# GmxMahdi/compute-raytracer

Hardware: AMD Instinct MI355X
Metric: Mrays/s at 3840x2160, 1024 spheres, 8 bounces (higher is better)
Workload: dtype f32; 1 GPU; C3: 3840x2160, 1024 spheres (seed 358), 8 bounces, constant sky, reference default camera/light; mode=fast, variant=0, rays_per_frame=46143642, frames_in_flight=4, parallelism=row-tiles x1

## Files before the change

### compute_raytracer_amd/csrc/rt_bvh.hip

```cpp
#include <algorithm>
#include <cmath>
#include <cstdlib>
#include <vector>

#include "rt_filter.h"

#define RT_BVH_KAPPA 6.103515625e-05f
#define RT_BVH_REV_DELTA 0.0051f
#define RT_BVH_REV_DELTA_REL 7.62939453125e-06f
#define RT_BVH_REV_SLACK 2.44140625e-04f
#define RT_BVH_REV_SLACK_ABS 4.76837158203125e-07f

#ifndef RT_BVH_GRAB
#define RT_BVH_GRAB 256u
#endif
#ifndef RT_BVH_TAIL_SMALL
#define RT_BVH_TAIL_SMALL 16
#endif
#ifndef RT_BVH_TAIL_SERIAL
#define RT_BVH_TAIL_SERIAL 12
#endif
#ifndef RT_BVH_TAIL_LARGE
#define RT_BVH_TAIL_LARGE 28
#endif

namespace rtk {

__host__ __device__ inline uint32_t bvh_lds_l0(uint32_t n_nodes, uint32_t base) {
    uint32_t l0 = 1024u;
    const uint32_t need = (4u * (n_nodes + 1u) + 2u) / 3u;
    if (base + l0 < need) l0 = need - base;
    return (l0 + 15u) & ~15u;
}
__host__ __device__ inline uint32_t bvh_gap_waves(uint32_t n_nodes, uint32_t waves) {
    const uint32_t k = (bvh_lds_l0(n_nodes, 0u) - 1024u) / 512u;
    return k < waves ? k : waves;
}
__host__ __device__ constexpr uint32_t bvh_list_bytes(bool nlds, uint32_t cap) { return nlds ? 128u * (cap + 1u) : 256u * cap; }
__host__ __device__ inline uint32_t bvh_lds_lists(uint32_t n_nodes, uint32_t base) {
    const uint32_t l0 = bvh_lds_l0(n_nodes, base);
    return 4u * (base + l0) - base + 16u * ((n_nodes + 4u) & ~3u);
}

__global__ void bvh_fill_leaves(float4* rec, const uint32_t* link, uint32_t n_nodes, const float4* geo_f) {
    const uint32_t i = blockIdx.x * blockDim.x + threadIdx.x;
    if (i >= n_nodes) return;
    const uint32_t l = link[i];
    if (l & 0x80000000u) rec[i] = geo_f[l & 0x7FFFFFFFu];
}

__device__ __forceinline__ double wave_max_f64(double v) {
#pragma unroll
    for (int off = 32; off > 0; off >>= 1) v = fmax(v, __shfl_xor(v, off, 64));
    return v;
}
__device__ __forceinline__ double wave_min_f64(double v) {
#pragma unroll
    for (int off = 32; off > 0; off >>= 1) v = fmin(v, __shfl_xor(v, off, 64));
    return v;
}

__global__ __launch_bounds__(256) void bvh_refit(float4* __restrict__ rec, const uint32_t* __restrict__ link,
                                                  uint32_t n_nodes, const float* __restrict__ records) {
    const uint32_t node = blockIdx.x * 4u + (threadIdx.x >> 6), lane = threadIdx.x & 63u;
    if (node >= n_nodes) return;
    const uint32_t lk = link[node];
    if (lk & 0x80000000u) return;
    const uint32_t first = node + 1u, end = lk >> 2;
    auto sphere = [&](uint32_t j, double c[3], double& r) -> bool {
        if (j >= end) return false;
        const uint32_t l = link[j];
        if (!(l & 0x80000000u)) return false;
        const float* s = records + 8u * (size_t)(l & 0x7FFFFFFFu);
        for (int a = 0; a < 3; ++a) { const double v = (double)s[a]; c[a] = v == v ? v : 0.0; }
        const double rv = fabs((double)s[7]);
        r = rv == rv ? rv : 0.0;
        return true;
    };
    auto radius_at = [&](const double P[3], double far[3]) -> double {
        double best = -1.0, bc[3] = {0.0, 0.0, 0.0};
        for (uint32_t j = first + lane; j < end; j += 64u) {
            double c[3], r;
            if (!sphere(j, c, r)) continue;
            const double dx = c[0] - P[0], dy = c[1] - P[1], dz = c[2] - P[2];
            const double d = sqrt(dx * dx + dy * dy + dz * dz) + r;
            if (d > best) { best = d; bc[0] = c[0]; bc[1] = c[1]; bc[2] = c[2]; }
        }
        const double R = wave_max_f64(best);
        const uint64_t who = __ballot(best == R);
        const int src = who ? (int)__builtin_ctzll(who) : 0;
        for (int a = 0; a < 3; ++a) far[a] = __shfl(bc[a], src, 64);
        return R;
    };
    double mn[3] = {INFINITY, INFINITY, INFINITY}, mx[3] = {-INFINITY, -INFINITY, -INFINITY};
    for (uint32_t j = first + lane; j < end; j += 64u) {
        double c[3], r;
        if (!sphere(j, c, r)) continue;
        for (int a = 0; a < 3; ++a) { mn[a] = fmin(mn[a], c[a] - r); mx[a] = fmax(mx[a], c[a] + r); }
    }
    double P[3];
    for (int a = 0; a < 3; ++a) P[a] = 0.5 * (wave_min_f64(mn[a]) + wave_max_f64(mx[a]));
    double far[3];
    double Rp = radius_at(P, far);
    for (int it = 0; it < 32; ++it) {
        const double sx = far[0] - P[0], sy = far[1] - P[1], sz = far[2] - P[2];
        const double len = sqrt(sx * sx + sy * sy + sz * sz);
        if (!(len > 1e-12)) break;
        const double Q[3] = {P[0] + sx / len * 0.05 * Rp, P[1] + sy / len * 0.05 * Rp, P[2] + sz / len * 0.05 * Rp};
        double farq[3];
        const double Rq = radius_at(Q, farq);
        if (!(Rq < Rp)) break;
        P[0] = Q[0]; P[1] = Q[1]; P[2] = Q[2]; Rp = Rq;
        far[0] = farq[0]; far[1] = farq[1]; far[2] = farq[2];
    }
    const float C[3] = {(float)P[0], (float)P[1], (float)P[2]};
    const double Cd[3] = {(double)C[0], (double)C[1], (double)C[2]};
    double unused[3];
    double R = radius_at(Cd, unused);
    R *= RT_BVH_SIGMA;
    const double c2 = Cd[0] * Cd[0] + Cd[1] * Cd[1] + Cd[2] * Cd[2];
    const double k = c2 * (1.0 - (double)RT_FILTER_EPS) - R * R * (1.0 + (double)RT_FILTER_KAPPA);
    if (lane == 0)
        rec[node] = make_float4(C[0] * RT_FILTER_SCALE, C[1] * RT_FILTER_SCALE, C[2] * RT_FILTER_SCALE,
                                (float)(k * (double)RT_FILTER_SCALE2));
}

#ifdef RT_BVH_COUNT
#define g_steps steps_acc
__device__ unsigned long long g_wave_clock[3 * 8192];
#endif
__device__ __forceinline__ float min0(float b) {
    float d; asm("v_min_f32 %0, 0, %1" : "=v"(d) : "v"(b)); return d;
}

__device__ __forceinline__ void exact_any_order(v3 center, float r2, int s, v3 o, v3 d, float fa, float ta,
                                                float& nearest, int& idx) {
    const v3 oc = sub(o, center);
    const float b = 2.0f * dot(d, oc);
    const float c = dot(oc, oc) - r2;
    const float disc = b * b - fa * c;
    if (disc > 0.0f && b < 0.0f) {
        const float t = (-b - sqrtf(disc)) / ta;
        if (t > 0.001f && (t < nearest || (t == nearest && idx >= 0 && s < idx))) {
            nearest = t;
            idx = s;
        }
    }
}

__device__ __forceinline__ void reversed_shadow_walk(bool shadow, v3 L, float light_l1, v3 P, v3 s, v3& wo, v3& wd, float& madd) {
    const v3 dl = sub(P, L);
    const float l1 = (__builtin_fabsf(dl.x) + __builtin_fabsf(dl.y)) + __builtin_fabsf(dl.z);
    const float la = l1 + light_l1;
    const float delta = __builtin_fmaf(la, RT_BVH_REV_DELTA_REL, RT_BVH_REV_DELTA);
    const float lb = l1 + delta;
    const float slack = __builtin_fmaf(lb * lb, RT_BVH_REV_SLACK, (la * la) * RT_BVH_REV_SLACK_ABS);
    if (shadow) {
        wo = V(__builtin_fmaf(delta, s.x, P.x), __builtin_fmaf(delta, s.y, P.y), __builtin_fmaf(delta, s.z, P.z));
        wd = V(-s.x, -s.y, -s.z);
        madd = slack;
    }
}

#define RT_BVH_DEC_DELTA 0.0050011f
#define RT_BVH_DEC_REL 9.5367431640625e-07f
__device__ __forceinline__ bool shadow_decided(v3 L, float light_l1, v3 s, float len, v3 c, float r2) {
    const float a2 = dot(s, s);
    const v3 oc = sub(L, c);
    const float b = 2.0f * dot(s, oc);
    const float cc = dot(oc, oc) - r2;
    const float disc = b * b - (4.0f * a2) * cc;
    if (!(disc > 0.0f && b < 0.0f)) return false;
    const float tk = (-b - sqrtf(disc)) / (2.0f * a2);
    const float d_a = __builtin_fmaf(len + light_l1, RT_BVH_DEC_REL, RT_BVH_DEC_DELTA);
    const float l_lo = len * (1.0f - RT_BVH_DEC_REL);
    return tk > 0.001f && tk < 9999.0f && tk + d_a <= l_lo;
}

template <bool SGN, bool NLDS, int CAP, bool ROOMY>
__device__ __forceinline__ void trace_bvh(const uint32_t tail, const float4* __restrict__ R, const uint32_t* __restrict__ L, uint32_t n,
                                          const float4* __restrict__ geo, uint32_t* slot, unsigned long long* best,
                                          uint32_t& i, v3 o, v3 d, v3 wo, v3 wd, float madd, float& nearest, int& idx
#ifdef RT_BVH_COUNT
                                          , uint32_t& steps_acc
#endif
                                          ) {
    const float a = dot(wd, wd);
    const float inv = __builtin_amdgcn_rsqf(a) * (1.0f + RT_BVH_KAPPA);
    const v3 h = V(wd.x * inv, wd.y * inv, wd.z * inv);
    const v3 os = V(wo.x * RT_FILTER_SCALE, wo.y * RT_FILTER_SCALE, wo.z * RT_FILTER_SCALE);
    const v3 m = V(-2.0f * os.x, -2.0f * os.y, -2.0f * os.z);
    const float p = dot(h, os);
    const float q = __builtin_fmaf(-madd, RT_FILTER_SCALE2, dot(os, os) * (1.0f - RT_FILTER_EPS));
    constexpr bool CLAMPED = SGN && NLDS;
    constexpr float kT = 2.168404344971009e-19f;
    constexpr float kT2 = 4.70197740328915e-38f;
    const v3 hs = V(h.x * kT, h.y * kT, h.z * kT);
    const v3 ms = V(m.x * kT2, m.y * kT2, m.z * kT2);
    const float ps = -p * kT, qs = q * kT2;
    typedef __attribute__((address_space(3))) uint32_t* lds_u32_w;
    typedef __attribute__((address_space(3))) uint16_t* lds_u16_w;
    const uint32_t wa0 = (uint32_t)(uintptr_t)slot;
    uint32_t wa = wa0;

    constexpr bool L16 = NLDS;
    typedef __attribute__((address_space(3))) const uint16_t* lds_u16;
    typedef __attribute__((address_space(3))) const uint32_t* lds_u32r;
    auto drain = [&]() {
        const uint32_t lane = threadIdx.x & 63u;
        const uint32_t cnt = L16 ? (wa - wa0) >> 7 : (wa - wa0) >> 8;
        uint32_t* const pool = slot - lane;
        const uint32_t top = wa0 - 2u * lane + 128u * (uint32_t)(CAP + 1);
        uint32_t total = 0;
        uint32_t lim = cnt;
        uint32_t again = 0;
        best[lane] = ((unsigned long long)__float_as_uint(nearest) << 32) | (unsigned long long)(uint32_t)idx;
      for (;;) {
        if (L16) {
            total = 0;
            uint32_t kstop = 0;
            bool stopped = false;
#pragma unroll
            for (int k = CAP - 1; k >= 0; --k) {
                const uint64_t m = __ballot((uint32_t)k < lim);
                if (m == 0ull) continue;
                const uint32_t need = (uint32_t)__popcll(m);
                if (!stopped && 4u * (total + need) > 128u * (uint32_t)(CAP + 1 - k)) { stopped = true; kstop = (uint32_t)k + 1u; }
                if (stopped) continue;
                uint32_t e = 0;
                if ((uint32_t)k < lim) e = *(lds_u16)(uintptr_t)(wa0 + 128u * (uint32_t)k);
                const uint32_t pos = total + __builtin_amdgcn_mbcnt_hi((uint32_t)(m >> 32), __builtin_amdgcn_mbcnt_lo((uint32_t)m, 0u));
                if ((uint32_t)k < lim) *(lds_u32_w)(uintptr_t)(top - 4u - 4u * pos) = (lane << 24) | e;
                total += need;
                asm volatile("" : "+s"(total));
            }
            again = stopped ? 1u : 0u;
            if (stopped) lim = lim < kstop ? lim : kstop;
        } else {
        for (uint32_t k = 0;; ++k) {
            const uint64_t m = __ballot(k < cnt);
            if (m == 0ull) break;
            uint32_t e = 0;
            if (k < cnt) e = slot[k * 64u];
            const uint32_t pos = total + (uint32_t)__popcll(m & ((1ull << lane) - 1ull));
            if (k < cnt) pool[pos] = (lane << 24) | (e & 0x00FFFFFFu);
            total += (uint32_t)__popcll(m);
        }
        }
        for (uint32_t i = lane; __ballot(i < total) != 0ull; i += 64u) {
#ifdef RT_BVH_COUNT
            if (RT_BVH_COUNT == 4) g_steps += lane == 0u ? 1u : 0u;
            if (RT_BVH_COUNT == 5) g_steps += i < total ? 1u : 0u;
#endif
            const uint32_t e = i < total ? (L16 ? *(lds_u32r)(uintptr_t)(top - 4u - 4u * i) : pool[i]) : (lane << 24);
            const int owner = (int)(e >> 24);
            const int si = (int)(e & 0x00FFFFFFu);
            typedef float f4r __attribute__((ext_vector_type(4)));
            f4r gr;
            asm volatile("global_load_dwordx4 %0, %1, %2" : "=&v"(gr) : "v"((uint32_t)si << 4), "s"(geo) : "memory");
            const v3 oo = V(__shfl(o.x, owner, 64), __shfl(o.y, owner, 64), __shfl(o.z, owner, 64));
            const v3 od = V(__shfl(d.x, owner, 64), __shfl(d.y, owner, 64), __shfl(d.z, owner, 64));
            if (i < total) {
                float a2 = dot(od, od);
                asm volatile("s_waitcnt vmcnt(0)" : "+v"(gr), "+v"(a2) : : "memory");
                const float4 g = make_float4(gr.x, gr.y, gr.z, gr.w);
                const v3 oc = sub(oo, V(g.x, g.y, g.z));
                const float b = 2.0f * dot(od, oc);
                const float c = dot(oc, oc) - g.w;
                const float disc = b * b - (4.0f * a2) * c;
                if (disc > 0.0f && b < 0.0f) {
                    const float t = (-b - sqrtf(disc)) / (2.0f * a2);
                    if (t > 0.001f && t < 9999.0f)
                        atomicMin(&best[owner], ((unsigned long long)__float_as_uint(t) << 32) | (unsigned long long)(uint32_t)si);
                }
            }
        }
        if (!L16 || __builtin_amdgcn_readfirstlane((int)again) == 0) break;
      }
        __builtin_amdgcn_fence(__ATOMIC_ACQ_REL, "wavefront");
        const unsigned long long r = best[lane];
        nearest = __uint_as_float((uint32_t)(r >> 32));
        idx = (int)(uint32_t)r;
        wa = wa0;
    };

    typedef __attribute__((address_space(3))) const uint32_t* lds_u32;
    typedef float f4v __attribute__((ext_vector_type(4)));
    typedef __attribute__((address_space(3))) const f4v* lds_f4;
    const uint32_t l0 = NLDS ? (uint32_t)(uintptr_t)L : 0u;
    auto fetch = [&](uint32_t j, float4& g, uint32_t& lk) {
        if (NLDS) {
            const f4v gv = *(lds_f4)(uintptr_t)j;
            lk = *(lds_u32)(uintptr_t)(j >> 2);
            g = make_float4(gv.x, gv.y, gv.z, gv.w);
        } else {
            lk = *reinterpret_cast<const uint32_t*>(reinterpret_cast<const char*>(L) + j);
            g = *reinterpret_cast<const float4*>(reinterpret_cast<const char*>(R) + 4u * (size_t)j);
        }
    };
    auto passes = [&](const float4& g) -> bool {
        if (CLAMPED) {
            float nb;
            const float part = fma_vvv(hs.y, g.y, fma_vvv(hs.x, g.x, ps));
            asm("v_fma_f32 %0, %1, %2, %3 clamp" : "=v"(nb) : "v"(hs.z), "v"(g.z), "v"(part));
            const float cp = fma_vvv(ms.z, g.z, fma_vvv(ms.y, g.y, fma_vvv(ms.x, g.x, g.w)));
            return __builtin_fmaf(nb, nb, -qs) > cp;
        } else {
            const float b = fnma_vvv(h.z, g.z, fnma_vvv(h.y, g.y, fnma_vvv(h.x, g.x, p)));
            const float cp = fma_vvv(m.z, g.z, fma_vvv(m.y, g.y, fma_vvv(m.x, g.x, g.w)));
            const float bm = SGN ? min0(b) : b;
            return __builtin_fmaf(bm, bm, -q) > cp;
        }
    };
    auto append = [&](uint32_t lk) {
        if (L16) {
            *(lds_u16_w)(uintptr_t)wa = (uint16_t)lk;
            asm("v_add_u32_e32 %0, 0x80, %0" : "+v"(wa));
        } else if (NLDS) {
            *(lds_u32_w)(uintptr_t)wa = lk;
            asm("v_add_u32_e32 %0, 0x100, %0" : "+v"(wa));
        } else {
            *(lds_u32_w)(uintptr_t)wa = lk;
            wa += 256u;
        }
    };
    const uint32_t jn = NLDS ? 4u * (4u * n + l0) : 4u * n;
    uint32_t j = NLDS ? 4u * (4u * i + l0) : 4u * i;
    const uint64_t walking0 = __ballot(j != jn);
    uint64_t walking = walking0;
    float4 g;
    uint32_t lk;
    fetch(j, g, lk);
    while (walking != 0ull) {
#ifdef RT_BVH_COUNT
        if (RT_BVH_COUNT == 1) g_steps += (threadIdx.x & 63u) == 0u ? 2u : 0u;
#endif
#pragma unroll
        for (int k = 0; k < 4; ++k) {
            const bool pass = passes(g);
            const bool leaf = (int)lk < 0;
#ifdef RT_BVH_COUNT
            if (RT_BVH_COUNT == 2) g_steps += j != jn ? 1u : 0u;
            if (RT_BVH_COUNT == 6) g_steps += leaf ? 1u : 0u;
            if (RT_BVH_COUNT == 7) g_steps += (!leaf && pass) ? 1u : 0u;
            if (RT_BVH_COUNT == 8) g_steps += (!leaf && lk != j) ? 1u : 0u;
#endif
            const uint32_t here = lk;
            j = (leaf || pass) ? j + (NLDS ? 16u : 4u) : lk;
            fetch(j, g, lk);
            if (leaf && pass) append(here);
        }
        if (__builtin_expect(__ballot(wa >= wa0 + (L16 ? 128u : 256u) * (uint32_t)(CAP - 3)) != 0ull, 0)) {
            drain();
            if (!ROOMY) fetch(j, g, lk);
        }
        walking = __ballot(j != jn);
        if (walking != walking0 && (uint32_t)__builtin_popcountll(walking) < tail) break;
    }
    drain();
    i = NLDS ? ((j >> 2) - l0) >> 2 : j >> 2;
}

inline bool lds_fits(size_t k, size_t bytes) { return k * ((bytes + 1279u) / 1280u) <= 128u; }
template <int WAVES, bool SGN, bool NLDS, int CAP, bool FLAT>
__global__ __launch_bounds__(64 * WAVES, WAVES == 16 ? 4 : 6) void bvh_pixels(const RtFrameArgs A) {
    extern __shared__ float4 lds[];
    const uint32_t n = A.bvh_nodes;
    const uint32_t n4 = (n + 4u) & ~3u;
    char* const lds_b = reinterpret_cast<char*>(lds);
    const uint32_t base = (uint32_t)(uintptr_t)lds;
    const uint32_t l0off = bvh_lds_l0(n, base);
    uint32_t* sL = reinterpret_cast<uint32_t*>(lds_b + (NLDS ? l0off : 0u));
    float4* sR = reinterpret_cast<float4*>(lds_b + (NLDS ? 4u * (base + l0off) - base : 0u));
    uint32_t* lists = reinterpret_cast<uint32_t*>(lds_b + (NLDS ? bvh_lds_lists(n, base) : 1024u));
    (void)n4;
    if (NLDS && base != 0u) { report_fault(A.rays, 1ull); return; }
    if (NLDS)
        for (uint32_t i = threadIdx.x; i <= n; i += 64 * WAVES) {
            float4 r = A.bvh_rec[i];
            if (SGN) r.w *= 4.70197740328915e-38f;
            sR[i] = r;
            const uint32_t lk = A.bvh_link[i];
            sL[i] = (int)lk < 0 ? lk : 4u * (lk + (uint32_t)(uintptr_t)sL);
        }
    const float4* R = NLDS ? sR : A.bvh_rec;
    const uint32_t* L = NLDS ? sL : A.bvh_link;
    const uint32_t lane = threadIdx.x & 63u;
    const uint32_t wave = (uint32_t)__builtin_amdgcn_readfirstlane((int)(threadIdx.x >> 6));
    constexpr uint32_t kListBytes = bvh_list_bytes(NLDS, (uint32_t)CAP);
    uint32_t* slot = reinterpret_cast<uint32_t*>(reinterpret_cast<char*>(lists) + wave * kListBytes + lane * (NLDS ? 2u : 4u));
    const uint32_t gapw = NLDS ? bvh_gap_waves(n, (uint32_t)WAVES) : 0u;
    unsigned long long* best = wave < gapw ? reinterpret_cast<unsigned long long*>(lds_b + 1024u) + wave * 64u
                                           : reinterpret_cast<unsigned long long*>(reinterpret_cast<char*>(lists) + WAVES * kListBytes) + (wave - gapw) * 64u;
    float* lut = reinterpret_cast<float*>(lds_b);
    for (uint32_t i = threadIdx.x; i < 256u; i += 64 * WAVES) lut[i] = (float)i / 255.0f;
    __syncthreads();

    const Scene sc = unpack_scene(A);
    v3 sky_c = V(0.0f, 0.0f, 0.0f);
    if (FLAT) {
        const v3 c = texel(A.face[0], 1, 1, 0, 0, lut);
        sky_c = V(__int_as_float(__builtin_amdgcn_readfirstlane(__float_as_int(c.x))),
                  __int_as_float(__builtin_amdgcn_readfirstlane(__float_as_int(c.y))),
                  __int_as_float(__builtin_amdgcn_readfirstlane(__float_as_int(c.z))));
    }
    auto flat_sky = [&](v3 r) -> v3 {
        const float z = (r.x * 0.0f + r.y * 0.0f) + r.z * 0.0f;
        return V(sky_c.x + z, sky_c.y + z, sky_c.z + z);
    };
    const float light_l1 = (__builtin_fabsf(sc.lightPos.x) + __builtin_fabsf(sc.lightPos.y)) + __builtin_fabsf(sc.lightPos.z);
    const uint32_t tiles_x = (A.W + 7u) / 8u;
    const uint32_t total = A.n_local_tiles * tiles_x * 64u;
    uint32_t cur = 0, end = 0;
    uint32_t chunk_ty = 0, chunk_tx = 0, chunk_first = ~0u;
    constexpr uint32_t kGrab = RT_BVH_GRAB;
    const uint32_t plenty = gridDim.x * (uint32_t)WAVES * 64u * 16u;
    uint32_t grab = 64u, trips = 0u;
    bool exhausted = false;
#ifdef RT_BVH_COUNT
    const uint64_t clk0 = wall_clock64();
    uint64_t clk_x = 0;
#endif

    bool active = false, shadow = false;
    uint32_t opix = 0, bounce = 0, nrays = 0;
    v3 ro = V(0, 0, 0), rd = V(0, 0, 1), color = V(1, 1, 1), fog = V(0, 0, 0);
    v3 normal = V(0, 0, 1), sdir = V(0, 0, 1), albedo = V(0, 0, 0);
    float dist = 0.0f, affect = 1.0f, sum = 0.0f, distance = 1.0f;
    uint32_t node = n;
    float t = 9999.0f;
    int idx = -1;

    for (;;) {
        ++trips;
        uint64_t idle = __ballot(!active);
        while (idle && !exhausted) {
            if (cur == end) {
                if (trips <= 2u && total - min(end, total) > plenty) grab = min(grab * 2u, kGrab);
                else if (trips > 8u) grab = 64u;
                trips = 0u;
                uint32_t base = 0;
#ifdef RT_BVH_COUNT
                const uint64_t clk_a = wall_clock64();
#endif
                if (lane == 0) base = atomicAdd(&A.qctrl[2], grab);
                base = __builtin_amdgcn_readfirstlane(base);
#ifdef RT_BVH_COUNT
                if (RT_BVH_COUNT == 14) nrays += lane == 0u ? 1u : 0u;
                if (RT_BVH_COUNT == 15) nrays += lane == 0u ? (uint32_t)(wall_clock64() - clk_a) : 0u;
#endif
                if (base >= total) {
                    exhausted = true;
#ifdef RT_BVH_COUNT
                    clk_x = wall_clock64();
#endif
                    break;
                }
                cur = base;
                end = min(base + grab, total);
            }
            if ((cur & 63u) == 0u || cur == chunk_first) {
                chunk_first = cur;
                chunk_ty = (cur >> 6) / tiles_x;
                chunk_tx = (cur >> 6) - chunk_ty * tiles_x;
            }
            const uint32_t tile_end = min(end, (cur & ~63u) + 64u);
            const uint32_t take = min((uint32_t)__popcll(idle), tile_end - cur);
            const uint32_t r = (uint32_t)__popcll(idle & ((1ull << lane) - 1ull));
            if (!active && r < take) {
                const uint32_t l = (cur + r) & 63u;
                const uint32_t ty = chunk_ty, tx = chunk_tx;
                const uint32_t x = tx * 8u + (l & 7u), row = l >> 3;
                const uint32_t y = (A.tile_first + ty * A.tile_step) * 8u + row;
                if (x < A.W && y < A.H) {
                    opix = (ty * 8u + row) * A.W + x;
                    ro = sc.cameraPos; rd = primary_dir(A, sc, x, y);
                    if (FLAT && sc.bounces == 0u) fog = scale(sc.minIntensity, flat_sky(rd));
                    color = V(1.0f, 1.0f, 1.0f); dist = 0.0f;
                    affect = 1.0f; sum = 0.0f; bounce = 0u;
                    shadow = false;
                    active = true;
                    node = 0u; t = 9999.0f; idx = -1;
                    if (sc.bounces == 0u) node = n;
                }
            }
            cur += take;
            idle = __ballot(!active);
        }
        if (__ballot(active) == 0ull) break;

        bool finished = active && sc.bounces == 0u;
        bool missed = false;
        const bool walking = node != n;
        v3 wo = ro, wd = shadow ? sdir : rd;
        float madd = 0.0f;
        if (SGN) reversed_shadow_walk(shadow, sc.lightPos, light_l1, ro, sdir, wo, wd, madd);
        else if (shadow) wo = sc.lightPos;
#ifdef RT_BVH_COUNT
        if (RT_BVH_COUNT == 3) nrays += lane == 0u ? 1u : 0u;
        trace_bvh<SGN, NLDS, CAP, WAVES == 16>(A.bvh_tail, R, L, n, A.geo, slot, best, node, shadow ? sc.lightPos : ro, shadow ? sdir : rd, wo, wd, madd, t, idx, nrays);
        if (walking && node == n) {
#else
        trace_bvh<SGN, NLDS, CAP, WAVES == 16>(A.bvh_tail, R, L, n, A.geo, slot, best, node, shadow ? sc.lightPos : ro, shadow ? sdir : rd, wo, wd, madd, t, idx);
        if (walking && node == n) {
            ++nrays;
#endif
            const float next = affect + sum;
            const bool shadow_done = shadow;
            bool decided = false;
            if (!shadow) {
                typedef float f3r __attribute__((ext_vector_type(3)));
                typedef float f4r __attribute__((ext_vector_type(4)));
                f4r hit_g;
                f3r hit_c;
                {
                    const uint32_t off = (uint32_t)(idx < 0 ? 0 : idx) << 4;
                    asm volatile("global_load_dwordx4 %0, %2, %3\n\tglobal_load_dwordx3 %1, %2, %4"
                                 : "=&v"(hit_g), "=&v"(hit_c) : "v"(off), "s"(A.geo), "s"(A.col) : "memory");
                }
                if (bounce == 0u) dist = idx >= 0 ? t : 0.0f;
                v3 sky = V(0, 0, 0);
                if (FLAT && (bounce == 0u || idx < 0)) sky = scale(sc.minIntensity, flat_sky(rd));
                if (FLAT && bounce == 0u) fog = sky;
                if (idx < 0) {
                    if (FLAT) color = divs(add(scale(sum, color), scale(affect, sky)), next);
                    else missed = true;
                    finished = true;
                }
                asm volatile("s_waitcnt vmcnt(0)" : "+v"(hit_g), "+v"(hit_c) : : "memory");
                if (idx >= 0) {
                    albedo = V(hit_c.x, hit_c.y, hit_c.z);
                    const v3 pos = add(ro, scale(t, rd));
                    const v3 centre = V(hit_g.x, hit_g.y, hit_g.z);
                    normal = normalize(sub(pos, centre));
                    ro = pos;
                    rd = normalize(reflect(rd, normal));
                    const v3 dl = sub(ro, sc.lightPos);
                    const float len = length(dl);
                    sdir = divs(dl, len);
                    distance = length_of_unit(sdir);
                    decided = shadow_decided(sc.lightPos, light_l1, sdir, len, centre, hit_g.w);
                    if (!decided) {
                        shadow = true;
                        node = 0u; t = 9999.0f; idx = -1;
                    }
#ifdef RT_BVH_COUNT
                    if (RT_BVH_COUNT == 16) nrays += decided ? 1u : 0u;
#else
                    if (decided) ++nrays;
#endif
                }
            }
            if (shadow_done || decided) {
                const float intensity = light_term(sc, ro, normal, sdir, distance, !decided && idx >= 0, t);
                const v3 blended = scale(intensity, albedo);
                color = divs(add(scale(sum, color), scale(affect, blended)), next);
                affect = affect / 2.0f;
                sum = next;
                ++bounce;
                shadow = false;
                finished = bounce >= sc.bounces;
                if (!finished) { node = 0u; t = 9999.0f; idx = -1; }
            }
        }
        if (finished) {
            if (FLAT) {
                reinterpret_cast<uint32_t*>(A.out)[opix] = compose_pixel_sky(fog, color, dist);
            } else {
                A.fin[2u * opix] = make_float4(color.x, color.y, color.z, __uint_as_float(__float_as_uint(dist) | (missed ? 0x80000000u : 0u)));
                if (missed && bounce != 0u) A.fin[2u * opix + 1u] = make_float4(rd.x, rd.y, rd.z, __uint_as_float(bounce));
            }
            active = false;
        }
    }
#ifdef RT_BVH_COUNT
    if (RT_BVH_COUNT == 9) nrays = lane == 0u ? (uint32_t)(wall_clock64() - (clk_x ? clk_x : clk0)) : 0u;
    if (RT_BVH_COUNT == 10) nrays = lane == 0u ? (uint32_t)(wall_clock64() - clk0) : 0u;
    if (RT_BVH_COUNT == 13 && lane == 0u) {
        const uint32_t w = (blockIdx.x * WAVES + wave) % 8192u;
        g_wave_clock[3 * w] = clk0; g_wave_clock[3 * w + 1] = clk_x ? clk_x : clk0; g_wave_clock[3 * w + 2] = wall_clock64();
    }
#endif
    count_rays(A.rays, nrays);
}

__global__ __launch_bounds__(256) void sky_resolve(const RtFrameArgs A) {
    __shared__ float lut[256];
    lut[threadIdx.x] = (float)threadIdx.x / 255.0f;
    __syncthreads();
    const Scene sc = unpack_scene(A);
    const uint32_t slots = A.n_local_tiles * 8u * A.W;
    for (uint32_t opix = blockIdx.x * 256u + threadIdx.x; opix < slots; opix += gridDim.x * 256u) {
        const uint32_t lrow = opix / A.W, x = opix - lrow * A.W;
        const uint32_t y = (A.tile_first + (lrow >> 3) * A.tile_step) * 8u + (lrow & 7u);
        if (y >= A.H) continue;
        const float4 r0 = A.fin[2u * opix];
        const v3 fog = scale(sc.minIntensity, cube_sample<2>(A, primary_dir(A, sc, x, y), lut));
        v3 color = V(r0.x, r0.y, r0.z);
        const float dist = __uint_as_float(__float_as_uint(r0.w) & 0x7FFFFFFFu);
        if ((__float_as_uint(r0.w) >> 31) != 0u) {
            float4 r1 = make_float4(0.0f, 0.0f, 0.0f, 0.0f);
            if (dist != 0.0f) r1 = A.fin[2u * opix + 1u];
            const uint32_t k = min(__float_as_uint(r1.w), sc.bounces);
            float affect = 1.0f, sum = 0.0f;
            for (uint32_t i = 0; i < k; ++i) { const float next = affect + sum; affect = affect / 2.0f; sum = next; }
            const float next = affect + sum;
            const v3 sky = k == 0u ? fog : scale(sc.minIntensity, cube_sample<2>(A, V(r1.x, r1.y, r1.z), lut));
            color = divs(add(scale(sum, color), scale(affect, sky)), next);
        }
        reinterpret_cast<uint32_t*>(A.out)[opix] = compose_pixel_sky(fog, color, dist);
    }
}

template <int WAVES, bool SGN, bool NLDS, int CAP, int TAIL>
hipError_t launch_bvh_as(const RtFrameArgs& a0, size_t lds, hipStream_t s) {
    RtFrameArgs a = a0;
    a.bvh_tail = (uint32_t)TAIL;
    if (TAIL == RT_BVH_TAIL_SMALL && a.grid_share <= 1u) a.bvh_tail = RT_BVH_TAIL_SERIAL;
    else if (TAIL == RT_BVH_TAIL_SMALL && a.n_local_tiles * 8u * a.W < (1u << 22)) a.bvh_tail = 12u;
#ifdef RT_BVH_DEV_ENV
    if (const char* e = getenv("RT355_BVH_TAIL")) a.bvh_tail = (uint32_t)atoi(e);
#endif
    auto k = a.sky_flat ? bvh_pixels<WAVES, SGN, NLDS, CAP, true> : bvh_pixels<WAVES, SGN, NLDS, CAP, false>;
    if (lds > 48u * 1024u) {
        hipError_t e = hipFuncSetAttribute(reinterpret_cast<const void*>(k), hipFuncAttributeMaxDynamicSharedMemorySize, (int)lds);
        if (e != hipSuccess) return e;
    }
    uint32_t per_cu = WAVES == 8 ? 3u : (WAVES == 12 ? 2u : 1u);
    while (per_cu > 1u && !lds_fits(per_cu, lds)) --per_cu;
    const uint32_t pixels = a.n_local_tiles * ((a.W + 7u) / 8u) * 64u;
    uint32_t blocks = 256u * (per_cu ? per_cu : 1u);
    if (a.grid_share > 1u) blocks = WAVES == 8 ? std::max(256u, blocks / a.grid_share) : std::max(1u, blocks / a.grid_share);
    const uint32_t need = (pixels + 64u * WAVES - 1u) / (64u * WAVES);
    if (blocks > need) blocks = need;
#ifdef RT_BVH_DEV_ENV
    if (const char* e = getenv("RT355_BVH_BLOCKS")) if (atoi(e) > 0) blocks = std::min((uint32_t)atoi(e), need);
    if (const char* e = getenv("RT355_BVH_LDS_PAD")) {
        lds += (size_t)atoi(e);
        (void)hipFuncSetAttribute(reinterpret_cast<const void*>(k), hipFuncAttributeMaxDynamicSharedMemorySize, (int)lds);
    }
#endif
    if (!a.sky_flat && !a.fin) return hipErrorInvalidValue;
    g_rt_kernel_id = !NLDS ? RT_KID_HIERARCHY_GLOBAL : (WAVES == 8 ? RT_KID_HIERARCHY_8 : (WAVES == 12 ? RT_KID_HIERARCHY_12 : RT_KID_HIERARCHY_16));
    hipLaunchKernelGGL(k, dim3(blocks), dim3(64 * WAVES), lds, s, a);
    if (!a.sky_flat) return rt_launch_sky_resolve(a, s);
    return hipGetLastError();
}

template <bool SGN>
hipError_t launch_bvh(const RtFrameArgs& a, hipStream_t s) {
    if (a.n_local_tiles == 0 || a.W == 0) return hipSuccess;
    constexpr int CAP = 12;
    const size_t nodes = (size_t)bvh_lds_lists(a.bvh_nodes, 0u);
    const size_t cap = 160u * 1024u;
    auto room = [&](uint32_t waves, uint32_t entries) {
        return nodes + (size_t)waves * bvh_list_bytes(true, entries) + (size_t)(waves - bvh_gap_waves(a.bvh_nodes, waves)) * 512u;
    };
#ifdef RT_BVH_DEV_ENV
    if (const char* e = getenv("RT355_BVH_CAP")) {
        if (atoi(e) == 16 && lds_fits(3u, room(8u, 16u))) return launch_bvh_as<8, SGN, true, 16, RT_BVH_TAIL_SMALL>(a, room(8u, 16u), s);
        if (atoi(e) == 8 && lds_fits(3u, room(8u, 8u))) return launch_bvh_as<8, SGN, true, 8, RT_BVH_TAIL_SMALL>(a, room(8u, 8u), s);
        if (atoi(e) == 10 && lds_fits(3u, room(8u, 10u))) return launch_bvh_as<8, SGN, true, 10, RT_BVH_TAIL_SMALL>(a, room(8u, 10u), s);
    }
#endif
    if (lds_fits(3u, room(8u, CAP))) return launch_bvh_as<8, SGN, true, CAP, RT_BVH_TAIL_SMALL>(a, room(8u, CAP), s);
    if (lds_fits(2u, room(12u, CAP))) return launch_bvh_as<12, SGN, true, CAP, RT_BVH_TAIL_SMALL>(a, room(12u, CAP), s);
    if (lds_fits(2u, room(12u, 6u))) return launch_bvh_as<12, SGN, true, 6, RT_BVH_TAIL_SMALL>(a, room(12u, 6u), s);
#ifdef RT_BVH_DEV_ENV
    if (const char* e = getenv("RT355_BVH_CAP")) {
        if (atoi(e) == 16 && room(16u, 16u) <= cap) return launch_bvh_as<16, SGN, true, 16, RT_BVH_TAIL_LARGE>(a, room(16u, 16u), s);
        if (atoi(e) == 8 && room(16u, 8u) <= cap) return launch_bvh_as<16, SGN, true, 8, RT_BVH_TAIL_LARGE>(a, room(16u, 8u), s);
        if (atoi(e) == 6 && room(16u, 6u) <= cap) return launch_bvh_as<16, SGN, true, 6, RT_BVH_TAIL_LARGE>(a, room(16u, 6u), s);
    }
#endif
    if (room(16u, CAP) <= cap)     return launch_bvh_as<16, SGN, true, CAP, RT_BVH_TAIL_LARGE>(a, room(16u, CAP), s);
    if (room(16u, 6u) <= cap)      return launch_bvh_as<16, SGN, true, 6, RT_BVH_TAIL_LARGE>(a, room(16u, 6u), s);
    return launch_bvh_as<8, SGN, false, 8, RT_BVH_TAIL_LARGE>(a, 1024u + 8u * ((size_t)bvh_list_bytes(false, 8u) + 512u), s);
}

}

#ifdef RT_BVH_COUNT
extern "C" __attribute__((visibility("default"))) int rt_debug_wave_clock(unsigned long long* dst, size_t n) {
    return (int)hipMemcpyFromSymbol(dst, HIP_SYMBOL(rtk::g_wave_clock), n * sizeof(unsigned long long));
}
#endif

hipError_t rt_launch_sky_resolve(const RtFrameArgs& a, hipStream_t s) {
    const uint32_t slots = a.n_local_tiles * 8u * a.W;
    if (slots == 0u) return hipSuccess;
    hipLaunchKernelGGL(rtk::sky_resolve, dim3(std::min((slots + 255u) / 256u, 256u * 8u)), dim3(256), 0, s, a);
    return hipGetLastError();
}

hipError_t rt_launch_bvh(const RtFrameArgs& a, hipStream_t s) {
    return a.signed_filter ? rtk::launch_bvh<true>(a, s) : rtk::launch_bvh<false>(a, s);
}

hipError_t rt_launch_bvh_refit(float4* rec, const uint32_t* link, uint32_t n_nodes, const float* records, hipStream_t s) {
    if (n_nodes == 0) return hipSuccess;
    hipLaunchKernelGGL(rtk::bvh_refit, dim3((n_nodes + 3u) / 4u), dim3(256), 0, s, rec, link, n_nodes, records);
    return hipGetLastError();
}

hipError_t rt_launch_bvh_fill(float4* rec, const uint32_t* link, uint32_t n_nodes, const float4* geo_f, hipStream_t s) {
    if (n_nodes == 0) return hipSuccess;
    hipLaunchKernelGGL(rtk::bvh_fill_leaves, dim3((n_nodes + 255u) / 256u), dim3(256), 0, s, rec, link, n_nodes, geo_f);
    return hipGetLastError();
}
```

Before: 32840 Mrays/s.

## Pack BVH link payload into low mantissa bits of node records in LDS

Adds a packed BVH layout that stores each node's link or leaf index in the low 8 bits of the x/y/z floats of its LDS record, with the leaf flag in z. Each traversal step then needs one 16-byte LDS load and a v_perm instead of a separate link load. To keep culling conservative, the sphere radius term is enlarged and the query slack is widened. Each block packs records at kernel start, votes on whether all records could be packed safely, and otherwise falls back to the unpacked path. The cost is extra setup work per block, a slightly looser cull test that can let more candidates through, and some duplicated code.

```diff
diff --git a/compute_raytracer_amd/csrc/rt_bvh.hip b/compute_raytracer_amd/csrc/rt_bvh.hip
--- a/compute_raytracer_amd/csrc/rt_bvh.hip
+++ b/compute_raytracer_amd/csrc/rt_bvh.hip
@@ -40,6 +40,33 @@
 __host__ __device__ inline uint32_t bvh_lds_lists(uint32_t n_nodes, uint32_t base) {
     const uint32_t l0 = bvh_lds_l0(n_nodes, base);
     return 4u * (base + l0) - base + 16u * ((n_nodes + 4u) & ~3u);
+}
+
+#define RT_BVH_PK_BASE 1024u
+#define RT_BVH_PK_MADD 1.0078125f
+#define RT_BVH_PK_EPS 3.814697265625e-06f
+#define RT_BVH_PK_LAMBDA_INV 513.0f
+#define RT_BVH_PK_MAX_GROWTH 0.25f
+__host__ __device__ inline bool bvh_pk_fits(uint32_t n_nodes) { return RT_BVH_PK_BASE + 16u * (n_nodes + 1u) <= 65536u; }
+__device__ __forceinline__ bool bvh_pack_record(const float4 r, uint32_t payload, bool leaf, float4& out) {
+    const uint32_t zb = __float_as_uint(r.z);
+    const float x = __uint_as_float((__float_as_uint(r.x) & ~0xFFu) | (payload & 0xFFu));
+    const float y = __uint_as_float((__float_as_uint(r.y) & ~0xFFu) | ((payload >> 8) & 0xFFu));
+    const float z = __uint_as_float(leaf ? ((zb & 0xFFu) != 0u ? zb : (zb | 1u)) : (zb & ~0xFFu));
+    const float dx = x - r.x, dy = y - r.y, dz = z - r.z;
+    const float up = 1.0000009537f;
+    const float d2 = ((dx * dx + dy * dy) + dz * dz) * up;
+    const float c2 = (r.x * r.x + r.y * r.y) + r.z * r.z;
+    const float c2p = (x * x + y * y) + z * z;
+    const float aw = __builtin_fabsf(r.w);
+    const float R2 = __builtin_fmaxf((c2 * (1.0f - RT_FILTER_EPS) - r.w) + (c2 + aw) * 4.76837158203125e-07f, 0.0f);
+    const float Rt = __builtin_sqrtf(R2) * up, dl = __builtin_sqrtf(d2) * up;
+    const float cover = ((2.0002f * dl) * Rt + RT_BVH_PK_LAMBDA_INV * d2) + (RT_BVH_PK_EPS * c2p + 5.9604644775390625e-07f * R2);
+    const float cd = (r.x * dx + r.y * dy) + r.z * dz;
+    out = make_float4(x, y, z, (r.w + 2.0f * cd) - cover);
+    const float big = 3.0e38f;
+    return __builtin_fabsf(r.x) < big && __builtin_fabsf(r.y) < big && __builtin_fabsf(r.z) < big && aw < big &&
+           __builtin_fabsf(out.w) < big && cover <= RT_BVH_PK_MAX_GROWTH * R2;
 }
 
 __global__ void bvh_fill_leaves(float4* rec, const uint32_t* link, uint32_t n_nodes, const float4* geo_f) {
@@ -177,7 +204,7 @@
     return tk > 0.001f && tk < 9999.0f && tk + d_a <= l_lo;
 }
 
-template <bool SGN, bool NLDS, int CAP, bool ROOMY>
+template <bool SGN, bool NLDS, int CAP, bool ROOMY, bool PK = false>
 __device__ __forceinline__ void trace_bvh(const uint32_t tail, const float4* __restrict__ R, const uint32_t* __restrict__ L, uint32_t n,
                                           const float4* __restrict__ geo, uint32_t* slot, unsigned long long* best,
                                           uint32_t& i, v3 o, v3 d, v3 wo, v3 wd, float madd, float& nearest, int& idx
@@ -191,7 +218,8 @@
     const v3 os = V(wo.x * RT_FILTER_SCALE, wo.y * RT_FILTER_SCALE, wo.z * RT_FILTER_SCALE);
     const v3 m = V(-2.0f * os.x, -2.0f * os.y, -2.0f * os.z);
     const float p = dot(h, os);
-    const float q = __builtin_fmaf(-madd, RT_FILTER_SCALE2, dot(os, os) * (1.0f - RT_FILTER_EPS));
+    const float q = PK ? __builtin_fmaf(-(madd * RT_BVH_PK_MADD), RT_FILTER_SCALE2, dot(os, os) * (1.0f - 1.5f * RT_FILTER_EPS))
+                       : __builtin_fmaf(-madd, RT_FILTER_SCALE2, dot(os, os) * (1.0f - RT_FILTER_EPS));
     constexpr bool CLAMPED = SGN && NLDS;
     constexpr float kT = 2.168404344971009e-19f;
     constexpr float kT2 = 4.70197740328915e-38f;
@@ -287,9 +315,16 @@
     typedef __attribute__((address_space(3))) const uint32_t* lds_u32;
     typedef float f4v __attribute__((ext_vector_type(4)));
     typedef __attribute__((address_space(3))) const f4v* lds_f4;
-    const uint32_t l0 = NLDS ? (uint32_t)(uintptr_t)L : 0u;
+    const uint32_t l0 = PK ? 0u : (NLDS ? (uint32_t)(uintptr_t)L : 0u);
+    const uint32_t r0 = PK ? (uint32_t)(uintptr_t)R : 0u;
+    uint32_t pk_sel = 0x0c0c0400u;
+    if (PK) asm volatile("" : "+v"(pk_sel));
     auto fetch = [&](uint32_t j, float4& g, uint32_t& lk) {
-        if (NLDS) {
+        if (PK) {
+            const f4v gv = *(lds_f4)(uintptr_t)j;
+            asm("v_perm_b32 %0, %1, %2, %3" : "=v"(lk) : "v"(gv.y), "v"(gv.x), "v"(pk_sel));
+            g = make_float4(gv.x, gv.y, gv.z, gv.w);
+        } else if (NLDS) {
             const f4v gv = *(lds_f4)(uintptr_t)j;
             lk = *(lds_u32)(uintptr_t)(j >> 2);
             g = make_float4(gv.x, gv.y, gv.z, gv.w);
@@ -324,8 +359,8 @@
             wa += 256u;
         }
     };
-    const uint32_t jn = NLDS ? 4u * (4u * n + l0) : 4u * n;
-    uint32_t j = NLDS ? 4u * (4u * i + l0) : 4u * i;
+    const uint32_t jn = PK ? r0 + 16u * n : (NLDS ? 4u * (4u * n + l0) : 4u * n);
+    uint32_t j = PK ? r0 + 16u * i : (NLDS ? 4u * (4u * i + l0) : 4u * i);
     const uint64_t walking0 = __ballot(j != jn);
     uint64_t walking = walking0;
     float4 g;
@@ -338,7 +373,7 @@
 #pragma unroll
         for (int k = 0; k < 4; ++k) {
             const bool pass = passes(g);
-            const bool leaf = (int)lk < 0;
+            const bool leaf = PK ? (__float_as_uint(g.z) & 0xFFu) != 0u : (int)lk < 0;
 #ifdef RT_BVH_COUNT
             if (RT_BVH_COUNT == 2) g_steps += j != jn ? 1u : 0u;
             if (RT_BVH_COUNT == 6) g_steps += leaf ? 1u : 0u;
@@ -358,12 +393,12 @@
         if (walking != walking0 && (uint32_t)__builtin_popcountll(walking) < tail) break;
     }
     drain();
-    i = NLDS ? ((j >> 2) - l0) >> 2 : j >> 2;
+    i = PK ? (j - r0) >> 4 : (NLDS ? ((j >> 2) - l0) >> 2 : j >> 2);
 }
 
 inline bool lds_fits(size_t k, size_t bytes) { return k * ((bytes + 1279u) / 1280u) <= 128u; }
-template <int WAVES, bool SGN, bool NLDS, int CAP, bool FLAT>
-__global__ __launch_bounds__(64 * WAVES, WAVES == 16 ? 4 : 6) void bvh_pixels(const RtFrameArgs A) {
+template <int WAVES, bool SGN, bool NLDS, int CAP, bool FLAT, bool PK>
+__device__ __forceinline__ bool bvh_frame(const RtFrameArgs& A) {
     extern __shared__ float4 lds[];
     const uint32_t n = A.bvh_nodes;
     const uint32_t n4 = (n + 4u) & ~3u;
@@ -371,11 +406,32 @@
     const uint32_t base = (uint32_t)(uintptr_t)lds;
     const uint32_t l0off = bvh_lds_l0(n, base);
     uint32_t* sL = reinterpret_cast<uint32_t*>(lds_b + (NLDS ? l0off : 0u));
-    float4* sR = reinterpret_cast<float4*>(lds_b + (NLDS ? 4u * (base + l0off) - base : 0u));
-    uint32_t* lists = reinterpret_cast<uint32_t*>(lds_b + (NLDS ? bvh_lds_lists(n, base) : 1024u));
+    float4* sR = reinterpret_cast<float4*>(lds_b + (PK ? RT_BVH_PK_BASE : (NLDS ? 4u * (base + l0off) - base : 0u)));
+    uint32_t* lists = reinterpret_cast<uint32_t*>(lds_b + (PK ? RT_BVH_PK_BASE + 16u * n4 : (NLDS ? bvh_lds_lists(n, base) : 1024u)));
     (void)n4;
-    if (NLDS && base != 0u) { report_fault(A.rays, 1ull); return; }
-    if (NLDS)
+    if (NLDS && base != 0u) { report_fault(A.rays, 1ull); return true; }
+    if (PK) {
+        volatile uint32_t* const vote = reinterpret_cast<volatile uint32_t*>(lds_b);
+        if (threadIdx.x == 0) *vote = 0u;
+        __syncthreads();
+        bool refused = false;
+        for (uint32_t i = threadIdx.x; i <= n; i += 64 * WAVES) {
+            const float4 r = A.bvh_rec[i];
+            const uint32_t lk = A.bvh_link[i];
+            const bool leaf = (int)lk < 0;
+            float4 pr;
+            const bool ok = bvh_pack_record(r, leaf ? (lk & 0xFFFFu) : RT_BVH_PK_BASE + 4u * lk, leaf, pr);
+            if (i == n) pr.w = r.w;
+            else refused = refused || !ok;
+            if (SGN) pr.w *= 4.70197740328915e-38f;
+            sR[i] = pr;
+        }
+        if (refused) *vote = 1u;
+        __syncthreads();
+        const bool any_refused = *vote != 0u;
+        __syncthreads();
+        if (any_refused) return false;
+    } else if (NLDS)
         for (uint32_t i = threadIdx.x; i <= n; i += 64 * WAVES) {
             float4 r = A.bvh_rec[i];
             if (SGN) r.w *= 4.70197740328915e-38f;
@@ -389,7 +445,7 @@
     const uint32_t wave = (uint32_t)__builtin_amdgcn_readfirstlane((int)(threadIdx.x >> 6));
     constexpr uint32_t kListBytes = bvh_list_bytes(NLDS, (uint32_t)CAP);
     uint32_t* slot = reinterpret_cast<uint32_t*>(reinterpret_cast<char*>(lists) + wave * kListBytes + lane * (NLDS ? 2u : 4u));
-    const uint32_t gapw = NLDS ? bvh_gap_waves(n, (uint32_t)WAVES) : 0u;
+    const uint32_t gapw = PK ? 0u : (NLDS ? bvh_gap_waves(n, (uint32_t)WAVES) : 0u);
     unsigned long long* best = wave < gapw ? reinterpret_cast<unsigned long long*>(lds_b + 1024u) + wave * 64u
                                            : reinterpret_cast<unsigned long long*>(reinterpret_cast<char*>(lists) + WAVES * kListBytes) + (wave - gapw) * 64u;
     float* lut = reinterpret_cast<float*>(lds_b);
@@ -498,10 +554,10 @@
         else if (shadow) wo = sc.lightPos;
 #ifdef RT_BVH_COUNT
         if (RT_BVH_COUNT == 3) nrays += lane == 0u ? 1u : 0u;
-        trace_bvh<SGN, NLDS, CAP, WAVES == 16>(A.bvh_tail, R, L, n, A.geo, slot, best, node, shadow ? sc.lightPos : ro, shadow ? sdir : rd, wo, wd, madd, t, idx, nrays);
+        trace_bvh<SGN, NLDS, CAP, WAVES == 16, PK>(A.bvh_tail, R, L, n, A.geo, slot, best, node, shadow ? sc.lightPos : ro, shadow ? sdir : rd, wo, wd, madd, t, idx, nrays);
         if (walking && node == n) {
 #else
-        trace_bvh<SGN, NLDS, CAP, WAVES == 16>(A.bvh_tail, R, L, n, A.geo, slot, best, node, shadow ? sc.lightPos : ro, shadow ? sdir : rd, wo, wd, madd, t, idx);
+        trace_bvh<SGN, NLDS, CAP, WAVES == 16, PK>(A.bvh_tail, R, L, n, A.geo, slot, best, node, shadow ? sc.lightPos : ro, shadow ? sdir : rd, wo, wd, madd, t, idx);
         if (walking && node == n) {
             ++nrays;
 #endif
@@ -582,6 +638,16 @@
     }
 #endif
     count_rays(A.rays, nrays);
+    return true;
+}
+
+template <int WAVES, bool SGN, bool NLDS, int CAP, bool FLAT, bool PK = false>
+__global__ __launch_bounds__(64 * WAVES, WAVES == 16 ? 4 : 6) void bvh_pixels(const RtFrameArgs A) {
+    if (PK) {
+        if (bvh_frame<WAVES, SGN, NLDS, CAP, FLAT, true>(A)) return;
+        __syncthreads();
+    }
+    bvh_frame<WAVES, SGN, NLDS, CAP, FLAT, false>(A);
 }
 
 __global__ __launch_bounds__(256) void sky_resolve(const RtFrameArgs A) {
@@ -612,7 +678,7 @@
     }
 }
 
-template <int WAVES, bool SGN, bool NLDS, int CAP, int TAIL>
+template <int WAVES, bool SGN, bool NLDS, int CAP, int TAIL, bool PK = false>
 hipError_t launch_bvh_as(const RtFrameArgs& a0, size_t lds, hipStream_t s) {
     RtFrameArgs a = a0;
     a.bvh_tail = (uint32_t)TAIL;
@@ -621,7 +687,7 @@
 #ifdef RT_BVH_DEV_ENV
     if (const char* e = getenv("RT355_BVH_TAIL")) a.bvh_tail = (uint32_t)atoi(e);
 #endif
-    auto k = a.sky_flat ? bvh_pixels<WAVES, SGN, NLDS, CAP, true> : bvh_pixels<WAVES, SGN, NLDS, CAP, false>;
+    auto k = a.sky_flat ? bvh_pixels<WAVES, SGN, NLDS, CAP, true, PK> : bvh_pixels<WAVES, SGN, NLDS, CAP, false, PK>;
     if (lds > 48u * 1024u) {
         hipError_t e = hipFuncSetAttribute(reinterpret_cast<const void*>(k), hipFuncAttributeMaxDynamicSharedMemorySize, (int)lds);
         if (e != hipSuccess) return e;
@@ -663,9 +729,14 @@
         if (atoi(e) == 10 && lds_fits(3u, room(8u, 10u))) return launch_bvh_as<8, SGN, true, 10, RT_BVH_TAIL_SMALL>(a, room(8u, 10u), s);
     }
 #endif
-    if (lds_fits(3u, room(8u, CAP))) return launch_bvh_as<8, SGN, true, CAP, RT_BVH_TAIL_SMALL>(a, room(8u, CAP), s);
-    if (lds_fits(2u, room(12u, CAP))) return launch_bvh_as<12, SGN, true, CAP, RT_BVH_TAIL_SMALL>(a, room(12u, CAP), s);
-    if (lds_fits(2u, room(12u, 6u))) return launch_bvh_as<12, SGN, true, 6, RT_BVH_TAIL_SMALL>(a, room(12u, 6u), s);
+    bool pk = bvh_pk_fits(a.bvh_nodes);
+    if (const char* e = getenv("RT355_BVH_PACKED")) pk = pk && atoi(e) != 0;
+    if (lds_fits(3u, room(8u, CAP)))
+        return pk ? launch_bvh_as<8, SGN, true, CAP, RT_BVH_TAIL_SMALL, true>(a, room(8u, CAP), s) : launch_bvh_as<8, SGN, true, CAP, RT_BVH_TAIL_SMALL>(a, room(8u, CAP), s);
+    if (lds_fits(2u, room(12u, CAP)))
+        return pk ? launch_bvh_as<12, SGN, true, CAP, RT_BVH_TAIL_SMALL, true>(a, room(12u, CAP), s) : launch_bvh_as<12, SGN, true, CAP, RT_BVH_TAIL_SMALL>(a, room(12u, CAP), s);
+    if (lds_fits(2u, room(12u, 6u)))
+        return pk ? launch_bvh_as<12, SGN, true, 6, RT_BVH_TAIL_SMALL, true>(a, room(12u, 6u), s) : launch_bvh_as<12, SGN, true, 6, RT_BVH_TAIL_SMALL>(a, room(12u, 6u), s);
 #ifdef RT_BVH_DEV_ENV
     if (const char* e = getenv("RT355_BVH_CAP")) {
         if (atoi(e) == 16 && room(16u, 16u) <= cap) return launch_bvh_as<16, SGN, true, 16, RT_BVH_TAIL_LARGE>(a, room(16u, 16u), s);
```

Result: slower. 30760 Mrays/s (-6.3%).
